# gauravchak/two_tower_models

Measured on AMD Instinct MI355X. Metric: user-item pairs/sec (in-batch softmax train step: fwd + zero_grad + bwd + dense-exact Adam), higher is better.
Workload: dtype f32

## Files before the change

### two_tower_models_amd/csrc/adam.hip

```cpp
#include <stdlib.h>

#include "common.hpp"

namespace tt {

constexpr int SWEEP_MAX_TABLES_DECL = 4;

constexpr int SWEEP_DEFAULT_PERSIST = 3;

struct AdamConst {
  float one_minus_b1, b2, one_minus_b2, eps, neg_step_size, inv_bc2_sqrt;
};

__device__ __forceinline__ AdamConst load_hyper(const double* __restrict__ h) {
  AdamConst c;
  c.one_minus_b1 = (float)(1.0 - h[1]);
  c.b2 = (float)h[2];
  c.one_minus_b2 = (float)(1.0 - h[2]);
  c.eps = (float)h[3];
  c.neg_step_size = (float)(-h[5]);
  c.inv_bc2_sqrt = (float)(1.0 / h[6]);
  return c;
}

// ... 352 lines not shown
  const AdamConst c = load_hyper(hyper);
  const unsigned n_chunks = tabs.first_chunk[tabs.n];
  __shared__ unsigned s_next[2];
  if (threadIdx.x == 0) s_next[0] = atomicAdd(&ctr[0], 1u);
  __syncthreads();
  unsigned ch = s_next[0];
  int par = 0;
  while (ch < n_chunks) {
    if (threadIdx.x == 0) s_next[par ^ 1] = atomicAdd(&ctr[0], 1u);
    int t = 0;
#pragma unroll
    for (int q = 1; q < SWEEP_MAX_TABLES; ++q)
      if (q < tabs.n && ch >= tabs.first_chunk[q]) t = q;
    float4* __restrict__ W = tabs.W[t];
    float4* __restrict__ M = tabs.M[t];
    float4* __restrict__ V = tabs.V[t];
    const int64_t n4 = tabs.n4[t];
    const int64_t base = (int64_t)(ch - tabs.first_chunk[t]) * (256 * ITERS) + threadIdx.x;
#pragma unroll UNR
    for (int k = 0; k < ITERS; ++k) {
      const int64_t i = base + (int64_t)k * 256;
      if (i >= n4) break;
      float4 p = sweep_load(W + i), m = sweep_load(M + i), v = sweep_load(V + i);
      adam_elem_zero_grad(p.x, m.x, v.x, c);
      adam_elem_zero_grad(p.y, m.y, v.y, c);
      adam_elem_zero_grad(p.z, m.z, v.z, c);
      adam_elem_zero_grad(p.w, m.w, v.w, c);
      sweep_store(p, W + i); sweep_store(m, M + i); sweep_store(v, V + i);
    }
    __syncthreads();
    par ^= 1;
    ch = s_next[par];
  }
  if (threadIdx.x == 0) {
    if (atomicAdd(&ctr[1], 1u) == gridDim.x - 1) {
      ctr[0] = 0;
      ctr[1] = 0;
      __threadfence();
    }
  }
}

struct SweepTablesMarked {
  SweepTables t;
  const unsigned* marks[SWEEP_MAX_TABLES];
  int sh[SWEEP_MAX_TABLES];
};
template <int ITERS, int PAIR>
__global__ __launch_bounds__(256) void adam_sweep_tables_marked_kernel(const SweepTablesMarked tm, const double* __restrict__ hyper,
                                                                       unsigned* __restrict__ ctr) {
  const AdamConst c = load_hyper(hyper);
  const unsigned n_chunks = tm.t.first_chunk[tm.t.n];
  __shared__ unsigned s_next[2];
  if (threadIdx.x == 0) s_next[0] = atomicAdd(&ctr[0], 1u);
  __syncthreads();
  unsigned ch = s_next[0];
  int par = 0;
  while (ch < n_chunks) {
    if (threadIdx.x == 0) s_next[par ^ 1] = atomicAdd(&ctr[0], 1u);
    const unsigned chu = __builtin_amdgcn_readfirstlane(ch);
    int t = 0;
#pragma unroll
    for (int q = 1; q < SWEEP_MAX_TABLES; ++q)
      if (q < tm.t.n && chu >= tm.t.first_chunk[q]) t = q;
    float4* __restrict__ W = tm.t.W[t];
    float4* __restrict__ M = tm.t.M[t];
    float4* __restrict__ V = tm.t.V[t];
    const int64_t n4 = tm.t.n4[t];
    const unsigned lc = chu - tm.t.first_chunk[t];
    const int sh = tm.sh[t];
    const int64_t r0 = (int64_t)lc * ((256 * ITERS) >> sh);
    const unsigned* __restrict__ mk = tm.marks[t];
    unsigned w0 = 0, w1 = 0, w2 = 0, w3 = 0;
    if (mk) {
      const unsigned* mw = mk + (r0 >> 5);
      w0 = mw[0]; w1 = mw[1]; w2 = mw[2]; w3 = mw[3];
    }
    const int64_t base = (int64_t)lc * (256 * ITERS) + threadIdx.x;
#pragma unroll
    for (int k = 0; k < ITERS; k += PAIR) {
      float4 p[PAIR], m[PAIR], v[PAIR];
      bool live[PAIR];
#pragma unroll
      for (int q = 0; q < PAIR; ++q) {
        const int64_t i = base + (int64_t)(k + q) * 256;
        const int64_t row = r0 + (((k + q) * 256 + (int)threadIdx.x) >> sh);
        const int wj = (int)((row >> 5) - (r0 >> 5));
        const unsigned word = wj == 0 ? w0 : wj == 1 ? w1 : wj == 2 ? w2 : w3;
        live[q] = i < n4 && !((word >> (row & 31)) & 1u);
      }
#pragma unroll
      for (int q = 0; q < PAIR; ++q) {
        const int64_t i = base + (int64_t)(k + q) * 256;
        if (live[q]) { p[q] = sweep_load(W + i); m[q] = sweep_load(M + i); v[q] = sweep_load(V + i); }
      }
#pragma unroll
      for (int q = 0; q < PAIR; ++q) {
        const int64_t i = base + (int64_t)(k + q) * 256;
        if (live[q]) {
          adam_elem_zero_grad(p[q].x, m[q].x, v[q].x, c);
          adam_elem_zero_grad(p[q].y, m[q].y, v[q].y, c);
          adam_elem_zero_grad(p[q].z, m[q].z, v[q].z, c);
          adam_elem_zero_grad(p[q].w, m[q].w, v[q].w, c);
          sweep_store(p[q], W + i); sweep_store(m[q], M + i); sweep_store(v[q], V + i);
        }
      }
    }
    __syncthreads();
    par ^= 1;
    ch = s_next[par];
  }
  if (threadIdx.x == 0) {
    if (atomicAdd(&ctr[1], 1u) == gridDim.x - 1) {
      ctr[0] = 0;
      ctr[1] = 0;
      __threadfence();
    }
  }
}

__global__ __launch_bounds__(256) void adam_mark_rows_kernel(const int64_t* __restrict__ ids, int64_t n_ids, int64_t n_rows,
                                                             unsigned* __restrict__ marks) {
  const int64_t i = (int64_t)blockIdx.x * 256 + threadIdx.x;
  if (i >= n_ids) return;
  const int64_t row = ids[i];
  if (row >= 0 && row < n_rows) atomicOr(&marks[row >> 5], 1u << (row & 31));
}

__global__ __launch_bounds__(256) void adam_sweep_scalar_kernel(float* __restrict__ W, float* __restrict__ M,
                                                                float* __restrict__ V, int64_t i0, int64_t n,
                                                                const double* __restrict__ hyper) {
  const AdamConst c = load_hyper(hyper);
  const int64_t stride = (int64_t)gridDim.x * blockDim.x;
  for (int64_t i = i0 + (int64_t)blockIdx.x * blockDim.x + threadIdx.x; i < n; i += stride) {
    float p = W[i], m = M[i], v = V[i];
    adam_elem_zero_grad(p, m, v, c);
    W[i] = p; M[i] = m; V[i] = v;
  }
}

__device__ __forceinline__ void replay_consts(AdamConst& c, const double* __restrict__ h, const float* __restrict__ tab,
                                              int64_t cap, int64_t j) {
  if (j < cap) {
    c.neg_step_size = tab[2 * j];
    c.inv_bc2_sqrt = tab[2 * j + 1];
  } else {
    double h5, h6;
    step_consts_from_doubles(h[0], h[1], h[2], (double)j, h5, h6);
    c.neg_step_size = (float)(-h5);
    c.inv_bc2_sqrt = (float)(1.0 / h6);
  }
}

template <int Q>
__device__ __forceinline__ void replay_row_q(float* __restrict__ W, float* __restrict__ M, float* __restrict__ V,
                                             int64_t row, int64_t dim, int32_t from, int32_t to,
                                             const double* __restrict__ hyper, const float* __restrict__ tab,
                                             int64_t cap, int lane) {
  AdamConst c = load_hyper(hyper);
  for (int64_t d0 = 0; d0 < dim; d0 += 64 * Q) {
    float p[Q], m[Q], v[Q];
    bool live = false;
#pragma unroll
    for (int q = 0; q < Q; ++q) {
      const int64_t d = d0 + lane + 64 * q;
      const int64_t at = row * dim + (d < dim ? d : dim - 1);
      p[q] = W[at]; m[q] = M[at]; v[q] = V[at];
      live = live || (d < dim && (m[q] != 0.f || v[q] != 0.f));
    }
    if (!__any(live)) continue;
    for (int32_t j = from + 1; j <= to; ++j) {
      replay_consts(c, hyper, tab, cap, j);
#pragma unroll
      for (int q = 0; q < Q; ++q) adam_elem_zero_grad(p[q], m[q], v[q], c);
    }
#pragma unroll
    for (int q = 0; q < Q; ++q) {
      const int64_t d = d0 + lane + 64 * q;
      if (d < dim) { W[row * dim + d] = p[q]; M[row * dim + d] = m[q]; V[row * dim + d] = v[q]; }
    }
  }
}
__device__ __forceinline__ void replay_row(float* __restrict__ W, float* __restrict__ M, float* __restrict__ V,
                                           int64_t row, int64_t dim, int32_t from, int32_t to,
                                           const double* __restrict__ hyper, const float* __restrict__ tab,
                                           int64_t cap, int lane) {
  from = __builtin_amdgcn_readfirstlane(from);
  to = __builtin_amdgcn_readfirstlane(to);
  if (dim <= 64) replay_row_q<1>(W, M, V, row, dim, from, to, hyper, tab, cap, lane);
  else if (dim <= 128) replay_row_q<2>(W, M, V, row, dim, from, to, hyper, tab, cap, lane);
  else replay_row_q<4>(W, M, V, row, dim, from, to, hyper, tab, cap, lane);
}

__global__ __launch_bounds__(256) void adam_catchup_ids_kernel(float* __restrict__ W, float* __restrict__ M,
                                                               float* __restrict__ V, int64_t n_rows, int64_t dim,
                                                               const int64_t* __restrict__ ids, int64_t n_ids,
                                                               int32_t* __restrict__ last_step,
                                                               const double* __restrict__ hyper, int offset,
                                                               const float* __restrict__ tab, int64_t cap) {
  const int64_t i = (int64_t)blockIdx.x * 4 + (threadIdx.x >> 6);
  if (i >= n_ids) return;
  const int lane = threadIdx.x & 63;
  const int64_t row = ids[i];
  if (row < 0 || row >= n_rows) return;
  const int32_t target = (int32_t)hyper[4] + offset;
  int32_t prev = 0;
  if (lane == 0) prev = atomicMax(&last_step[row], target);
  prev = __shfl(prev, 0, 64);
  if (prev >= target) return;
  replay_row(W, M, V, row, dim, prev, target, hyper, tab, cap, lane);
}

__global__ __launch_bounds__(256) void adam_catchup_plan_kernel(float* __restrict__ W, float* __restrict__ M,
                                                                float* __restrict__ V, int64_t n_rows, int64_t dim,
                                                                const int32_t* __restrict__ sorted_ids,
                                                                const int32_t* __restrict__ seg_begin,
                                                                const int32_t* __restrict__ n_unique,
                                                                int32_t* __restrict__ last_step,
                                                                const double* __restrict__ hyper, int offset, int mark,
                                                                const float* __restrict__ tab, int64_t cap) {
  const int64_t u = (int64_t)blockIdx.x * 4 + (threadIdx.x >> 6);
  if (u >= *n_unique) return;
  const int lane = threadIdx.x & 63;
  const int64_t row = sorted_ids[seg_begin[u]];
  if (row >= n_rows) return;
  const int32_t target = (int32_t)hyper[4] + offset;
  const int32_t prev = last_step[row];
  if (prev < target) replay_row(W, M, V, row, dim, prev, target, hyper, tab, cap, lane);
  if (lane == 0) last_step[row] = target + mark;
}

__global__ __launch_bounds__(256) void adam_flush_kernel(float* __restrict__ W, float* __restrict__ M,
                                                         float* __restrict__ V, int64_t n_rows, int64_t dim,
                                                         int32_t* __restrict__ last_step,
                                                         const double* __restrict__ hyper,
                                                         const float* __restrict__ tab, int64_t cap) {
  const int lane = threadIdx.x & 63;
  const int32_t target = (int32_t)hyper[4];
  const int64_t stride = (int64_t)gridDim.x * 4;
  for (int64_t row = (int64_t)blockIdx.x * 4 + (threadIdx.x >> 6); row < n_rows; row += stride) {
    const int32_t prev = last_step[row];
    if (prev >= target) continue;
    replay_row(W, M, V, row, dim, prev, target, hyper, tab, cap, lane);
    if (lane == 0) last_step[row] = target;
  }
}

constexpr int ADAM_BATCH = 64;
struct AdamBatch { tt_adam_tensor t[ADAM_BATCH]; };
__global__ __launch_bounds__(256) void adam_dense_kernel(const AdamBatch ts, const double* __restrict__ hyper) {
  const tt_adam_tensor t = ts.t[blockIdx.y];
  const AdamConst c = load_hyper(hyper);
  const int64_t stride = (int64_t)gridDim.x * blockDim.x;
  for (int64_t i = (int64_t)blockIdx.x * blockDim.x + threadIdx.x; i < t.n; i += stride) {
    float p = t.p[i], m = t.m[i], v = t.v[i];
    adam_elem(p, m, v, t.g[i], c);
    t.p[i] = p; t.m[i] = m; t.v[i] = v;
  }
}

__global__ __launch_bounds__(256) void pack_grads_kernel(const AdamBatch ts) {
  const tt_adam_tensor t = ts.t[blockIdx.y];
  const int64_t stride = (int64_t)gridDim.x * blockDim.x;
  for (int64_t i = (int64_t)blockIdx.x * blockDim.x + threadIdx.x; i < t.n; i += stride) t.p[i] = t.g[i];
}

__global__ __launch_bounds__(256) void copy_buffers_kernel(const AdamBatch ts) {
  const tt_adam_tensor t = ts.t[blockIdx.y];
  char* dst = reinterpret_cast<char*>(t.p);
  const char* src = reinterpret_cast<const char*>(t.g);
  const int64_t stride = (int64_t)gridDim.x * blockDim.x, i0 = (int64_t)blockIdx.x * blockDim.x + threadIdx.x;
  const bool vec = ((reinterpret_cast<uintptr_t>(dst) | reinterpret_cast<uintptr_t>(src)) & 15) == 0;
  const int64_t n16 = vec ? t.n / 16 : 0;
  for (int64_t i = i0; i < n16; i += stride) reinterpret_cast<uint4*>(dst)[i] = reinterpret_cast<const uint4*>(src)[i];
  for (int64_t i = n16 * 16 + i0; i < t.n; i += stride) dst[i] = src[i];
}

__global__ __launch_bounds__(256) void rowgrad_dense_kernel(const tt_grad_sources src, int64_t n_rows, int64_t dim,
                                                            const int32_t* __restrict__ sorted_ids,
                                                            const int32_t* __restrict__ perm,
                                                            const int32_t* __restrict__ seg_begin,
                                                            const int32_t* __restrict__ n_unique,
                                                            float* __restrict__ dense) {
  const int64_t u = (int64_t)blockIdx.x * 4 + (threadIdx.x >> 6);
  if (u >= *n_unique) return;
  const int lane = threadIdx.x & 63;
  const int32_t t0 = seg_begin[u], t1 = seg_begin[u + 1];
  const int64_t row = sorted_ids[t0];
  if (row >= n_rows) return;
  for (int64_t d = lane; d < dim; d += 64) {
    float g = 0.f;
    for (int32_t t = t0; t < t1; ++t) g += source_row(src, perm[t])[d];
    dense[row * dim + d] = g;
  }
}

static bool check_sources(const tt_grad_sources* s, int64_t n_ids, int64_t dim) {
  if (!s || s->n_sources < 1 || s->n_sources > TT_MAX_GRAD_SOURCES || s->first[0] != 0) return false;
  for (int k = 0; k < s->n_sources; ++k)
    if (!s->rows[k] || s->ld[k] < dim || s->first[k + 1] < s->first[k]) return false;
  return s->first[s->n_sources] == n_ids;
}

static int device_cu_count() {
  static int cached[64] = {0};
  int dev = 0;
  if (hipGetDevice(&dev) != hipSuccess || dev < 0 || dev >= 64) return 256;
  if (cached[dev] == 0) {
    int n = 0;
    cached[dev] = (hipDeviceGetAttribute(&n, hipDeviceAttributeMultiprocessorCount, dev) == hipSuccess && n > 0) ? n : 256;
  }
  return cached[dev];
}

static int launch_sweep(float* W, float* M, float* V, int64_t n_rows, int64_t dim, const double* hyper,
                        hipStream_t st, int n_wgs = 0) {
  int rc;
  const int64_t total = n_rows * dim;
  const bool vec = ((reinterpret_cast<uintptr_t>(W) | reinterpret_cast<uintptr_t>(M) | reinterpret_cast<uintptr_t>(V)) & 15) == 0;
  const int64_t n4 = vec ? total / 4 : 0;
  if (n4 > 0) {
    float4 *w4 = reinterpret_cast<float4*>(W), *m4 = reinterpret_cast<float4*>(M), *v4 = reinterpret_cast<float4*>(V);
    ProfScope prof("adam_sweep_kernel", st);
    unsigned* ctr = reinterpret_cast<unsigned*>(const_cast<double*>(hyper) + 7);
    unsigned grid = (unsigned)(device_cu_count() * SWEEP_DEFAULT_PERSIST);
    if (n_wgs > 0 && (unsigned)n_wgs < grid) grid = (unsigned)n_wgs;
    adam_sweep_persistent_kernel<4, 4><<<grid, 256, 0, st>>>(w4, m4, v4, n4, hyper, ctr);
    if ((rc = check_launch("adam_sweep_kernel"))) return rc;
  }
  if (n4 * 4 < total) {
    const int64_t rem = total - n4 * 4;
    const int64_t blocks = ceil_div(rem, 256) < 2048 ? ceil_div(rem, 256) : 2048;
    adam_sweep_scalar_kernel<<<(unsigned)blocks, 256, 0, st>>>(W, M, V, n4 * 4, total, hyper);
    if ((rc = check_launch("adam_sweep_scalar_kernel"))) return rc;
  }
  return 0;
}

}

using namespace tt;

extern "C" int tt_adam_advance(double* hyper, tt_stream_t stream) {
  if (!hyper) return fail_arg("tt_adam_advance: null pointer");
  adam_advance_kernel<<<1, 1, 0, S(stream)>>>(hyper, nullptr, 0);
  return check_launch("adam_advance_kernel");
}

extern "C" int64_t tt_adam_table_workspace_bytes(int64_t n_ids, int64_t dim) {
  if (n_ids <= 0 || dim <= 0) return 256;
  return round_up(n_ids * 3 * dim * 4, 256);
}

extern "C" int tt_adam_table(float* W, float* M, float* V, int64_t n_rows, int64_t dim, const double* hyper,
                             const tt_grad_sources* src, int64_t n_ids, const int32_t* sorted_ids,
                             const int32_t* perm, const int32_t* seg_begin, const int32_t* n_unique,
                             void* ws, int64_t ws_bytes, tt_stream_t stream) {
  if (!W || !M || !V || !hyper) return fail_arg("tt_adam_table: null pointer");
  if (n_rows <= 0 || dim <= 0 || n_ids < 0) return fail_arg("tt_adam_table: sizes");
  hipStream_t st = S(stream);
  int rc;
  if (n_ids > 0) {
    if (!sorted_ids || !perm || !seg_begin || !n_unique || !ws) return fail_arg("tt_adam_table: null plan");
    if (!check_sources(src, n_ids, dim)) return fail_arg("tt_adam_table: gradient sources");
    if (ws_bytes < tt_adam_table_workspace_bytes(n_ids, dim)) { set_error("tt_adam_table: workspace"); return TT_E_WORKSPACE; }
    adam_touched_kernel<false><<<(unsigned)ceil_div(n_ids, 4), 256, 0, st>>>(W, M, V, n_rows, dim, hyper, *src, sorted_ids, perm, seg_begin, n_unique, reinterpret_cast<float*>(ws), n_ids);
    if ((rc = check_launch("adam_touched_kernel"))) return rc;
  }
  if ((rc = launch_sweep(W, M, V, n_rows, dim, hyper, st))) return rc;
  if (n_ids > 0) {
    adam_writeback_kernel<<<(unsigned)ceil_div(n_ids, 4), 256, 0, st>>>(W, M, V, n_rows, dim, sorted_ids, seg_begin, perm, n_unique, reinterpret_cast<const float*>(ws), n_ids);
    if ((rc = check_launch("adam_writeback_kernel"))) return rc;
  }
  return 0;
}

extern "C" int tt_adam_table_stash(const float* W, const float* M, const float* V, int64_t n_rows, int64_t dim,
                                   int64_t n_ids, const int32_t* sorted_ids, const int32_t* perm,
                                   const int32_t* seg_begin, const int32_t* n_unique, void* side,
                                   int64_t side_bytes, tt_stream_t stream) {
  if (!W || !M || !V || !sorted_ids || !perm || !seg_begin || !n_unique || !side) return fail_arg("tt_adam_table_stash: null pointer");
  if (n_rows <= 0 || dim <= 0 || n_ids <= 0) return fail_arg("tt_adam_table_stash: sizes");
  if (side_bytes < tt_adam_table_workspace_bytes(n_ids, dim)) { set_error("tt_adam_table_stash: side buffer"); return TT_E_WORKSPACE; }
  adam_stash_kernel<<<(unsigned)ceil_div(n_ids, 4), 256, 0, S(stream)>>>(W, M, V, n_rows, dim, sorted_ids, seg_begin, perm, n_unique, reinterpret_cast<float*>(side), n_ids);
  return check_launch("adam_stash_kernel");
}

extern "C" int tt_adam_table_stash_ids(const float* W, const float* M, const float* V, int64_t n_rows, int64_t dim,
                                       const int64_t* ids, int64_t n_ids, void* side, int64_t side_bytes,
                                       tt_stream_t stream) {
  if (!W || !M || !V || !ids || !side) return fail_arg("tt_adam_table_stash_ids: null pointer");
  if (n_rows <= 0 || dim <= 0 || n_ids <= 0) return fail_arg("tt_adam_table_stash_ids: sizes");
  if (side_bytes < tt_adam_table_workspace_bytes(n_ids, dim)) { set_error("tt_adam_table_stash_ids: side buffer"); return TT_E_WORKSPACE; }
  adam_stash_ids_kernel<<<(unsigned)ceil_div(n_ids, 4), 256, 0, S(stream)>>>(W, M, V, n_rows, dim, ids, n_ids, reinterpret_cast<float*>(side));
  return check_launch("adam_stash_ids_kernel");
}

static int begin_ids_impl(double* hyper, float* tab, int64_t tab_steps, const tt_adam_stash_job* jobs, int32_t n_jobs, int planes,
                          tt_stream_t stream);

extern "C" int tt_adam_begin_ids(double* hyper, float* tab, int64_t tab_steps, const tt_adam_stash_job* jobs, int32_t n_jobs,
                                 tt_stream_t stream) {
  return begin_ids_impl(hyper, tab, tab_steps, jobs, n_jobs, 7, stream);
}

extern "C" int tt_adam_begin_ids_planes(double* hyper, float* tab, int64_t tab_steps, const tt_adam_stash_job* jobs, int32_t n_jobs,
                                        int32_t planes, tt_stream_t stream) {
  if (planes <= 0 || planes > 7) return fail_arg("tt_adam_begin_ids_planes: planes is a mask of 1 (p), 2 (m), 4 (v)");
  if (n_jobs > SWEEP_MAX_TABLES) return fail_arg("tt_adam_begin_ids_planes: at most 4 tables");
  return begin_ids_impl(hyper, tab, tab_steps, jobs, n_jobs, planes, stream);
}

static int begin_ids_impl(double* hyper, float* tab, int64_t tab_steps, const tt_adam_stash_job* jobs, int32_t n_jobs, int planes,
                          tt_stream_t stream) {
  if (!hyper || (n_jobs > 0 && !jobs) || n_jobs < 0) return fail_arg("tt_adam_begin_ids: null pointer");
  if (tab && tab_steps <= 0) return fail_arg("tt_adam_begin_ids: sizes");
  hipStream_t st = S(stream);
  if (n_jobs > SWEEP_MAX_TABLES) {
    int rc = tab ? tt_adam_advance_tab(hyper, tab, tab_steps, stream) : tt_adam_advance(hyper, stream);
    for (int i = 0; i < n_jobs && !rc; ++i)
      rc = tt_adam_table_stash_ids(jobs[i].W, jobs[i].M, jobs[i].V, jobs[i].n_rows, jobs[i].dim, jobs[i].ids, jobs[i].n_ids,
                                   jobs[i].side, jobs[i].side_bytes, stream);
    return rc;
  }
  StashJobs a{};
  a.n = n_jobs;
  unsigned blocks = 0;
  for (int i = 0; i < n_jobs; ++i) {
    const tt_adam_stash_job& j = jobs[i];
    if (!j.W || !j.M || !j.V || !j.ids || !j.side) return fail_arg("tt_adam_begin_ids: null pointer");
    if (j.n_rows <= 0 || j.dim <= 0 || j.n_ids <= 0) return fail_arg("tt_adam_begin_ids: sizes");
    if (j.side_bytes < tt_adam_table_workspace_bytes(j.n_ids, j.dim)) { set_error("tt_adam_begin_ids: side buffer"); return TT_E_WORKSPACE; }
    a.W[i] = j.W; a.M[i] = j.M; a.V[i] = j.V; a.ids[i] = j.ids; a.side[i] = reinterpret_cast<float*>(j.side);
    a.n_rows[i] = j.n_rows; a.dim[i] = j.dim; a.n_ids[i] = j.n_ids;
    a.first_block[i] = blocks;
    blocks += (unsigned)ceil_div(j.n_ids, 4);
  }
  for (int i = n_jobs; i <= SWEEP_MAX_TABLES; ++i) a.first_block[i] = blocks;
  adam_begin_ids_kernel<<<blocks + 1, 256, 0, st>>>(a, hyper, tab, tab ? tab_steps : 0, planes, planes & 1);
  return check_launch("adam_begin_ids_kernel");
}

extern "C" int tt_adam_table_sweep(float* W, float* M, float* V, int64_t n_rows, int64_t dim, const double* hyper,
                                   tt_stream_t stream) {
  if (!W || !M || !V || !hyper) return fail_arg("tt_adam_table_sweep: null pointer");
  if (n_rows <= 0 || dim <= 0) return fail_arg("tt_adam_table_sweep: sizes");
  return launch_sweep(W, M, V, n_rows, dim, hyper, S(stream));
}

extern "C" int tt_adam_tables_sweep(const tt_adam_tensor* tables, int32_t n_tables, const double* hyper, int32_t n_wgs,
                                    tt_stream_t stream) {
  if (!tables || !hyper) return fail_arg("tt_adam_tables_sweep: null pointer");
  if (n_tables <= 0 || n_tables > SWEEP_MAX_TABLES) return fail_arg("tt_adam_tables_sweep: 1..4 tables");
  hipStream_t st = S(stream);
  bool fused = n_tables > 1;
  SweepTables tabs{};
  unsigned chunks = 0;
  for (int t = 0; t < n_tables; ++t) {
    const tt_adam_tensor& d = tables[t];
    if (!d.p || !d.m || !d.v || d.n <= 0) return fail_arg("tt_adam_tables_sweep: descriptor");
    if (((reinterpret_cast<uintptr_t>(d.p) | reinterpret_cast<uintptr_t>(d.m) | reinterpret_cast<uintptr_t>(d.v)) & 15) || d.n % 4) fused = false;
    tabs.W[t] = reinterpret_cast<float4*>(d.p); tabs.M[t] = reinterpret_cast<float4*>(d.m); tabs.V[t] = reinterpret_cast<float4*>(d.v);
    tabs.n4[t] = d.n / 4;
    tabs.first_chunk[t] = chunks;
    const int64_t c = ceil_div(d.n / 4, 256 * 4);
    if (c + chunks >= (1ll << 32)) fused = false;
    chunks += (unsigned)c;
  }
  tabs.first_chunk[n_tables] = chunks;
  tabs.n = n_tables;
  static const int wgs_env = getenv("TT_SWEEP_WGS") ? atoi(getenv("TT_SWEEP_WGS")) : 0;
  const int want = getenv("TT_SWEEP_WGS") ? wgs_env : n_wgs;
  if (!fused) {
    for (int t = 0; t < n_tables; ++t) {
      const int rc = launch_sweep(tables[t].p, tables[t].m, tables[t].v, tables[t].n, 1, hyper, st, want);
      if (rc) return rc;
    }
    return 0;
  }
  unsigned* ctr = reinterpret_cast<unsigned*>(const_cast<double*>(hyper) + 7);
  unsigned grid = (unsigned)(device_cu_count() * SWEEP_DEFAULT_PERSIST);
  if (want > 0 && (unsigned)want < grid) grid = (unsigned)want;
  ProfScope prof("adam_sweep_kernel", st);
  adam_sweep_tables_kernel<4, 4><<<grid, 256, 0, st>>>(tabs, hyper, ctr);
  return check_launch("adam_sweep_tables_kernel");
}

extern "C" int64_t tt_adam_marks_words(int64_t n_rows) { return n_rows > 0 ? (n_rows + 31) / 32 + 4 : 4; }

extern "C" int tt_adam_mark_rows(const int64_t* ids, int64_t n_ids, int64_t n_rows, uint32_t* marks, int64_t marks_words,
                                 tt_stream_t stream) {
  if (!ids || !marks) return fail_arg("tt_adam_mark_rows: null pointer");
  if (n_ids <= 0 || n_rows <= 0) return fail_arg("tt_adam_mark_rows: sizes");
  if (marks_words < tt_adam_marks_words(n_rows)) { set_error("tt_adam_mark_rows: bitmap of %lld words < %lld", (long long)marks_words, (long long)tt_adam_marks_words(n_rows)); return TT_E_WORKSPACE; }
  hipStream_t st = S(stream);
  hipError_t e = hipMemsetAsync(marks, 0, (size_t)marks_words * 4, st);
  if (e != hipSuccess) { set_error("tt_adam_mark_rows: hipMemsetAsync: %s", hipGetErrorString(e)); return (int)e; }
  adam_mark_rows_kernel<<<(unsigned)ceil_div(n_ids, 256), 256, 0, st>>>(ids, n_ids, n_rows, marks);
  return check_launch("adam_mark_rows_kernel");
}

extern "C" int tt_adam_marked_supported(int64_t dim) {
  if (dim < 32 || dim > 4096 || (dim & (dim - 1))) return 0;
  return 1;
}

extern "C" int tt_adam_tables_sweep_marked(const tt_adam_tensor* tables, const int64_t* dims, const uint32_t* const* marks,
                                           int32_t n_tables, const double* hyper, int32_t n_wgs, tt_stream_t stream) {
  if (!tables || !dims || !marks || !hyper) return fail_arg("tt_adam_tables_sweep_marked: null pointer");
  if (n_tables <= 0 || n_tables > SWEEP_MAX_TABLES) return fail_arg("tt_adam_tables_sweep_marked: 1..4 tables");
  SweepTablesMarked tm{};
  unsigned chunks = 0;
  for (int t = 0; t < n_tables; ++t) {
    const tt_adam_tensor& d = tables[t];
    if (!d.p || !d.m || !d.v || d.n <= 0) return fail_arg("tt_adam_tables_sweep_marked: descriptor");
    if (!tt_adam_marked_supported(dims[t]) || d.n % dims[t]) return fail_arg("tt_adam_tables_sweep_marked: dim must be a power of two in [32, 4096]");
    if ((reinterpret_cast<uintptr_t>(d.p) | reinterpret_cast<uintptr_t>(d.m) | reinterpret_cast<uintptr_t>(d.v)) & 15)
      return fail_arg("tt_adam_tables_sweep_marked: 16-byte aligned tables");
    tm.t.W[t] = reinterpret_cast<float4*>(d.p); tm.t.M[t] = reinterpret_cast<float4*>(d.m); tm.t.V[t] = reinterpret_cast<float4*>(d.v);
    tm.t.n4[t] = d.n / 4;
    tm.t.first_chunk[t] = chunks;
    const int64_t c = ceil_div(d.n / 4, 256 * 4);
    if (c + chunks >= (1ll << 32)) return fail_arg("tt_adam_tables_sweep_marked: too many chunks");
    chunks += (unsigned)c;
    tm.marks[t] = marks[t];
    int sh = 0;
    while ((4ll << sh) < dims[t]) ++sh;
    tm.sh[t] = sh;
  }
  tm.t.first_chunk[n_tables] = chunks;
  tm.t.n = n_tables;
  static const int wgs_env = getenv("TT_SWEEP_WGS") ? atoi(getenv("TT_SWEEP_WGS")) : 0;
  const int want = getenv("TT_SWEEP_WGS") ? wgs_env : n_wgs;
  unsigned* ctr = reinterpret_cast<unsigned*>(const_cast<double*>(hyper) + 7);
  unsigned grid = (unsigned)(device_cu_count() * SWEEP_DEFAULT_PERSIST);
  if (want > 0 && (unsigned)want < grid) grid = (unsigned)want;
  hipStream_t st = S(stream);
  ProfScope prof("adam_sweep_kernel", st);
  adam_sweep_tables_marked_kernel<4, 2><<<grid, 256, 0, st>>>(tm, hyper, ctr);
  return check_launch("adam_sweep_tables_marked_kernel");
}

extern "C" int tt_stream_create_low_priority(void** out) {
  if (!out) return fail_arg("tt_stream_create_low_priority: null pointer");
  int least = 0, greatest = 0;
  hipError_t e = hipDeviceGetStreamPriorityRange(&least, &greatest);
  if (e != hipSuccess) { set_error("hipDeviceGetStreamPriorityRange: %s", hipGetErrorString(e)); return (int)e; }
  hipStream_t s;
  e = hipStreamCreateWithPriority(&s, hipStreamNonBlocking, least);
  if (e != hipSuccess) { set_error("hipStreamCreateWithPriority: %s", hipGetErrorString(e)); return (int)e; }
  *out = reinterpret_cast<void*>(s);
  return 0;
}
extern "C" int tt_stream_destroy(void* stream) {
  if (!stream) return 0;
  hipError_t e = hipStreamDestroy(reinterpret_cast<hipStream_t>(stream));
  if (e != hipSuccess) { set_error("hipStreamDestroy: %s", hipGetErrorString(e)); return (int)e; }
  return 0;
}

extern "C" int tt_adam_table_finish(float* W, float* M, float* V, int64_t n_rows, int64_t dim, const double* hyper,
                                    const tt_grad_sources* src, int64_t n_ids, const int32_t* sorted_ids,
                                    const int32_t* perm, const int32_t* seg_begin, const int32_t* n_unique,
                                    void* side, int64_t side_bytes, tt_stream_t stream) {
  if (!W || !M || !V || !hyper || !sorted_ids || !perm || !seg_begin || !n_unique)
    return fail_arg("tt_adam_table_finish: null pointer");
  if (n_rows <= 0 || dim <= 0 || n_ids <= 0) return fail_arg("tt_adam_table_finish: sizes");
  if (!check_sources(src, n_ids, dim)) return fail_arg("tt_adam_table_finish: gradient sources");
  if (side && side_bytes < tt_adam_table_workspace_bytes(n_ids, dim)) { set_error("tt_adam_table_finish: side buffer"); return TT_E_WORKSPACE; }
  hipStream_t st = S(stream);
  float* sd = reinterpret_cast<float*>(side);
  bool vec = dim % 4 == 0 && ((reinterpret_cast<uintptr_t>(W) | reinterpret_cast<uintptr_t>(M) | reinterpret_cast<uintptr_t>(V) |
                               reinterpret_cast<uintptr_t>(side)) & 15) == 0;
  for (int k = 0; vec && k < src->n_sources; ++k)
    vec = (reinterpret_cast<uintptr_t>(src->rows[k]) & 15) == 0 && src->ld[k] % 4 == 0;
  if (vec) {
    if (dim <= 64) adam_finish_kernel<16><<<(unsigned)ceil_div(n_ids, 16), 256, 0, st>>>(W, M, V, n_rows, dim, hyper, *src, sorted_ids, perm, seg_begin, n_unique, sd, n_ids);
    else if (dim <= 128) adam_finish_kernel<32><<<(unsigned)ceil_div(n_ids, 8), 256, 0, st>>>(W, M, V, n_rows, dim, hyper, *src, sorted_ids, perm, seg_begin, n_unique, sd, n_ids);
    else adam_finish_kernel<64><<<(unsigned)ceil_div(n_ids, 4), 256, 0, st>>>(W, M, V, n_rows, dim, hyper, *src, sorted_ids, perm, seg_begin, n_unique, sd, n_ids);
    return check_launch("adam_finish_kernel");
  }
  if (!side) return fail_arg("tt_adam_table_finish: marked rows (side == NULL) need dim % 4 == 0 and 16-byte aligned operands");
  adam_touched_kernel<true><<<(unsigned)ceil_div(n_ids, 4), 256, 0, st>>>(W, M, V, n_rows, dim, hyper, *src, sorted_ids, perm, seg_begin, n_unique, sd, n_ids);
  int rc = check_launch("adam_touched_kernel");
  if (rc) return rc;
  adam_writeback_kernel<<<(unsigned)ceil_div(n_ids, 4), 256, 0, st>>>(W, M, V, n_rows, dim, sorted_ids, seg_begin, perm, n_unique, sd, n_ids);
  return check_launch("adam_writeback_kernel");
}

extern "C" int tt_adam_tables_finish(const tt_adam_finish_job* jobs, int32_t n_jobs, const double* hyper, tt_stream_t stream) {
  if (!jobs || !hyper || n_jobs <= 0) return fail_arg("tt_adam_tables_finish: null pointer");
  bool one = n_jobs <= SWEEP_MAX_TABLES;
  int lpr = 0;
  for (int i = 0; i < n_jobs; ++i) {
    const tt_adam_finish_job& j = jobs[i];
    if (!j.W || !j.M || !j.V || !j.src || !j.sorted_ids || !j.perm || !j.seg_begin || !j.n_unique)
      return fail_arg("tt_adam_tables_finish: null pointer");
    if (j.n_rows <= 0 || j.dim <= 0 || j.n_ids <= 0) return fail_arg("tt_adam_tables_finish: sizes");
    if (!check_sources(j.src, j.n_ids, j.dim)) return fail_arg("tt_adam_tables_finish: gradient sources");
    if (j.side && j.side_bytes < tt_adam_table_workspace_bytes(j.n_ids, j.dim)) { set_error("tt_adam_tables_finish: side buffer"); return TT_E_WORKSPACE; }
    bool vec = j.dim % 4 == 0 && ((reinterpret_cast<uintptr_t>(j.W) | reinterpret_cast<uintptr_t>(j.M) | reinterpret_cast<uintptr_t>(j.V) |
                                   reinterpret_cast<uintptr_t>(j.side)) & 15) == 0;
    for (int k = 0; vec && k < j.src->n_sources; ++k)
      vec = (reinterpret_cast<uintptr_t>(j.src->rows[k]) & 15) == 0 && j.src->ld[k] % 4 == 0;
    const int cls = j.dim <= 64 ? 16 : j.dim <= 128 ? 32 : 64;
    if (!vec || (lpr && cls != lpr)) one = false;
    lpr = lpr ? lpr : cls;
  }
  if (!one) {
    for (int i = 0; i < n_jobs; ++i) {
      const tt_adam_finish_job& j = jobs[i];
      int rc = tt_adam_table_finish(j.W, j.M, j.V, j.n_rows, j.dim, hyper, j.src, j.n_ids, j.sorted_ids, j.perm, j.seg_begin,
                                    j.n_unique, j.side, j.side_bytes, stream);
      if (rc) return rc;
    }
    return 0;
  }
// ... 168 lines not shown
```

### two_tower_models_amd/csrc/attention_mfma.hip

```cpp
#include <stdlib.h>

#include "common.hpp"

namespace tt {

typedef float f32x16 __attribute__((ext_vector_type(16)));

constexpr int HP = 64;

__device__ __forceinline__ int arow(int e, int h) { return (e & 3) + 8 * (e >> 2) + 4 * h; }

template <int DH>
struct AttnLds {
  static constexpr int LD = DH + 4;
  static constexpr int MAT = HP * LD;
};

template <int DH>
__device__ __forceinline__ void stage(float* dst, const float* __restrict__ src, int64_t ld, int H, float scale, int lane) {
  constexpr int C4 = DH / 4, LD = DH + 4;
#pragma unroll
  for (int it = 0; it < HP * C4 / 64; ++it) {
    const int f = it * 64 + lane;
    const int row = f / C4, c4 = f % C4;
    const bool ok = row < H;
    const float* p = src + (int64_t)(ok ? row : H - 1) * ld + 4 * c4;
    const float x0 = p[0], x1 = p[1], x2 = p[2], x3 = p[3];
    const float4 v = make_float4(ok ? x0 * scale : 0.f, ok ? x1 * scale : 0.f, ok ? x2 * scale : 0.f, ok ? x3 * scale : 0.f);
    *reinterpret_cast<float4*>(dst + row * LD + 4 * c4) = v;
  }
}

template <int DH>
__device__ __forceinline__ void load_bfrag(float4 (&bf)[DH / 8], const float* __restrict__ src, int64_t ld, int row,
                                           int H, float scale, int h) {
  const bool ok = row < H;
  const float* p = src + (int64_t)(ok ? row : H - 1) * ld + 4 * h;
#pragma unroll
  for (int g = 0; g < DH / 8; ++g) {
    const float x0 = p[8 * g], x1 = p[8 * g + 1], x2 = p[8 * g + 2], x3 = p[8 * g + 3];
    bf[g] = make_float4(ok ? x0 * scale : 0.f, ok ? x1 * scale : 0.f, ok ? x2 * scale : 0.f, ok ? x3 * scale : 0.f);
  }
}
template <int DH>
__device__ __forceinline__ f32x16 nt_tile_rb(const float* A, int a0, const float4 (&bf)[DH / 8], int r, int h) {
  constexpr int LD = DH + 4;
  f32x16 acc;
#pragma unroll
  for (int e = 0; e < 16; ++e) acc[e] = 0.f;
  const float* ap = A + (a0 + r) * LD + 4 * h;
#pragma unroll
  for (int g = 0; g < DH / 8; ++g) {
    const float4 a = *reinterpret_cast<const float4*>(ap + 8 * g);
    acc = __builtin_amdgcn_mfma_f32_32x32x2f32(a.x, bf[g].x, acc, 0, 0, 0);
    acc = __builtin_amdgcn_mfma_f32_32x32x2f32(a.y, bf[g].y, acc, 0, 0, 0);
    acc = __builtin_amdgcn_mfma_f32_32x32x2f32(a.z, bf[g].z, acc, 0, 0, 0);
    acc = __builtin_amdgcn_mfma_f32_32x32x2f32(a.w, bf[g].w, acc, 0, 0, 0);
  }
  return acc;
}

template <int DH>
__device__ __forceinline__ void py_accum(f32x16 (&out)[(DH + 31) / 32], const f32x16& G, const float* Y, int y0,
                                         int r, int h) {
  constexpr int LD = DH + 4, TD = (DH + 31) / 32;
#pragma unroll
  for (int e = 0; e < 16; ++e) {
    const float* yrow = Y + (y0 + (e & 3) + 8 * (e >> 2) + 4 * h) * LD;
#pragma unroll
    for (int d = 0; d < TD; ++d) {
      const int col = 32 * d + r;
      const float yv = (DH % 32 == 0 || col < DH) ? yrow[col] : 0.f;
      out[d] = __builtin_amdgcn_mfma_f32_32x32x2f32(G[e], yv, out[d], 0, 0, 0);
    }
  }
}

template <int DH>
__device__ __forceinline__ void store_rows(float* __restrict__ dst, int64_t ld, const f32x16 (&t)[(DH + 31) / 32],
                                           int x0, int H, float scale, int r, int h) {
  constexpr int TD = (DH + 31) / 32;
#pragma unroll
  for (int d = 0; d < TD; ++d) {
    const int col = 32 * d + r;
    if (col >= DH) continue;
#pragma unroll
    for (int e = 0; e < 16; ++e) {
      const int row = x0 + arow(e, h);
      if (row < H) dst[(int64_t)row * ld + col] = t[d][e] * scale;
    }
  }
}

template <int DH, int WAVES>
__global__ __launch_bounds__(64 * WAVES, (WAVES == 4 ? 2 : 1)) void attn_fwd_mfma_kernel(const float* __restrict__ qkv, int64_t n_pairs,
                                                                   int H, int D, int heads,
                                                                   float* __restrict__ ctx, float* __restrict__ lse) {
  using L = AttnLds<DH>;
  constexpr int TD = (DH + 31) / 32;
  extern __shared__ __attribute__((aligned(16))) char smem_raw[];
  const int lane = threadIdx.x & 63, wave = threadIdx.x >> 6, r = lane & 31, h = lane >> 5;
  const int64_t pair = (int64_t)blockIdx.x * WAVES + wave;
  if (pair >= n_pairs) return;
  float* Ks = reinterpret_cast<float*>(smem_raw) + wave * 2 * L::MAT;
  float* Vs = Ks + L::MAT;
  const int64_t b = pair / heads, hd = pair % heads;
  const float* base = qkv + b * H * 3 * (int64_t)D + hd * DH;
  const float scale = 1.0f / sqrtf((float)DH);
  constexpr int C4 = DH / 4, NST = HP * C4 / 64;
  float4 kst[NST], vst[NST];
#pragma unroll
  for (int it = 0; it < NST; ++it) {
    const int f = it * 64 + lane, row = f / C4, c4 = f % C4;
    const float* pr = base + (int64_t)(row < H ? row : H - 1) * (3 * D) + 4 * c4;
    kst[it] = *reinterpret_cast<const float4*>(pr + D);
    vst[it] = *reinterpret_cast<const float4*>(pr + 2 * D);
  }
  float4 qf0[DH / 8], qf1[DH / 8];
  load_bfrag<DH>(qf0, base, 3 * D, r, H, scale, h);
  load_bfrag<DH>(qf1, base, 3 * D, 32 + r, H, scale, h);
#pragma unroll
  for (int it = 0; it < NST; ++it) {
    const int f = it * 64 + lane, row = f / C4, c4 = f % C4;
    const bool ok = row < H;
    float4 kv = kst[it], vv = vst[it];
    const float m = ok ? 1.f : 0.f;
    kv.x *= m; kv.y *= m; kv.z *= m; kv.w *= m;
    vv.x *= m; vv.y *= m; vv.z *= m; vv.w *= m;
    *reinterpret_cast<float4*>(Ks + row * L::LD + 4 * c4) = kv;
    *reinterpret_cast<float4*>(Vs + row * L::LD + 4 * c4) = vv;
  }
  __builtin_amdgcn_wave_barrier();

  float* out = ctx + b * H * (int64_t)D + hd * DH;
  auto query_tile = [&](int it, const float4 (&qf)[DH / 8]) {
    f32x16 st[2];
    float mx = -3.0e38f;
#pragma unroll
    for (int jt = 0; jt < 2; ++jt) {
      st[jt] = nt_tile_rb<DH>(Ks, jt * 32, qf, r, h);
#pragma unroll
      for (int e = 0; e < 16; ++e) {
        const bool valid = jt * 32 + arow(e, h) < H;
        st[jt][e] = valid ? st[jt][e] : -3.0e38f;
        mx = fmaxf(mx, st[jt][e]);
      }
    }
    mx = fmaxf(mx, __shfl_xor(mx, 32, 64));
    float l = 0.f;
#pragma unroll
    for (int jt = 0; jt < 2; ++jt)
#pragma unroll
      for (int e = 0; e < 16; ++e) {
        st[jt][e] = __expf(st[jt][e] - mx);
        l += st[jt][e];
      }
    l += __shfl_xor(l, 32, 64);
    const float inv = 1.0f / l;
    f32x16 o[TD];
#pragma unroll
    for (int d = 0; d < TD; ++d)
#pragma unroll
      for (int e = 0; e < 16; ++e) o[d][e] = 0.f;
#pragma unroll
    for (int jt = 0; jt < 2; ++jt) {
#pragma unroll
      for (int e = 0; e < 16; ++e) st[jt][e] *= inv;
      py_accum<DH>(o, st[jt], Vs, jt * 32, r, h);
    }
    store_rows<DH>(out, D, o, it * 32, H, 1.f, r, h);
    const int i = it * 32 + r;
    if (h == 0 && i < H) lse[(b * heads + hd) * H + i] = mx + __logf(l);
  };
  query_tile(0, qf0);
  query_tile(1, qf1);
}

template <int DH, int WAVES>
__global__ __launch_bounds__(64 * WAVES, (WAVES == 4 ? 2 : 1)) void attn_bwd_mfma_kernel(const float* __restrict__ qkv,
                                                                   const float* __restrict__ lse,
                                                                   const float* __restrict__ d_ctx, int64_t n_pairs,
                                                                   int H, int D, int heads,
                                                                   float* __restrict__ d_qkv) {
  using L = AttnLds<DH>;
  constexpr int TD = (DH + 31) / 32;
  constexpr int PER_WAVE = 2 * L::MAT + 2 * HP;
  extern __shared__ __attribute__((aligned(16))) char smem_raw[];
  const int lane = threadIdx.x & 63, wave = threadIdx.x >> 6, r = lane & 31, h = lane >> 5;
  const int64_t pair = (int64_t)blockIdx.x * WAVES + wave;
  if (pair >= n_pairs) return;
  float* M0 = reinterpret_cast<float*>(smem_raw) + wave * PER_WAVE;
  float* M1 = M0 + L::MAT;
  float* Ls = M1 + L::MAT;
  float* Ds = Ls + HP;
  const int64_t b = pair / heads, hd = pair % heads;
  const float* base = qkv + b * H * 3 * (int64_t)D + hd * DH;
  const float* gbase = d_ctx + b * H * (int64_t)D + hd * DH;
  const float scale = 1.0f / sqrtf((float)DH);
  float* Ks = M0;
  float* Vs = M1;
  stage<DH>(Ks, base + D, 3 * D, H, 1.f, lane);
  stage<DH>(Vs, base + 2 * D, 3 * D, H, 1.f, lane);
  Ls[lane] = (lane < H) ? lse[(b * heads + hd) * H + lane] : 3.0e38f;
  __builtin_amdgcn_wave_barrier();
  float* obase = d_qkv + b * H * 3 * (int64_t)D + hd * DH;

#pragma unroll
  for (int it = 0; it < 2; ++it) {
    const int i = it * 32 + r;
    const float li = Ls[i];
    float4 qf[DH / 8], gf[DH / 8];
    load_bfrag<DH>(qf, base, 3 * D, i, H, scale, h);
    load_bfrag<DH>(gf, gbase, D, i, H, 1.f, h);
    f32x16 pt[2], dpt[2];
    float dl = 0.f;
#pragma unroll
    for (int jt = 0; jt < 2; ++jt) {
      pt[jt] = nt_tile_rb<DH>(Ks, jt * 32, qf, r, h);
      dpt[jt] = nt_tile_rb<DH>(Vs, jt * 32, gf, r, h);
#pragma unroll
      for (int e = 0; e < 16; ++e) {
        const bool valid = jt * 32 + arow(e, h) < H;
        pt[jt][e] = valid ? __expf(pt[jt][e] - li) : 0.f;
        dl = fmaf(pt[jt][e], dpt[jt][e], dl);
      }
    }
    dl += __shfl_xor(dl, 32, 64);
    if (h == 0) Ds[i] = dl;
    f32x16 dq[TD];
#pragma unroll
    for (int d = 0; d < TD; ++d)
#pragma unroll
      for (int e = 0; e < 16; ++e) dq[d][e] = 0.f;
#pragma unroll
    for (int jt = 0; jt < 2; ++jt) {
#pragma unroll
      for (int e = 0; e < 16; ++e) pt[jt][e] *= (dpt[jt][e] - dl);
      py_accum<DH>(dq, pt[jt], Ks, jt * 32, r, h);
    }
    store_rows<DH>(obase, 3 * D, dq, it * 32, H, scale, r, h);
  }
  __builtin_amdgcn_wave_barrier();

  float* Qs = M0;
  float* Gs = M1;
  stage<DH>(Qs, base, 3 * D, H, scale, lane);
  stage<DH>(Gs, gbase, D, H, 1.f, lane);
  __builtin_amdgcn_wave_barrier();
#pragma unroll
  for (int jt = 0; jt < 2; ++jt) {
    const bool jvalid = jt * 32 + r < H;
    float4 kf[DH / 8], vf[DH / 8];
    load_bfrag<DH>(kf, base + D, 3 * D, jt * 32 + r, H, 1.f, h);
    load_bfrag<DH>(vf, base + 2 * D, 3 * D, jt * 32 + r, H, 1.f, h);
    f32x16 dv[TD], dk[TD];
#pragma unroll
    for (int d = 0; d < TD; ++d)
#pragma unroll
      for (int e = 0; e < 16; ++e) { dv[d][e] = 0.f; dk[d][e] = 0.f; }
#pragma unroll
    for (int it = 0; it < 2; ++it) {
      f32x16 p = nt_tile_rb<DH>(Qs, it * 32, kf, r, h);
      f32x16 dp = nt_tile_rb<DH>(Gs, it * 32, vf, r, h);
      const float* lrow = Ls + it * 32 + 4 * h;
      const float* drow = Ds + it * 32 + 4 * h;
#pragma unroll
      for (int q = 0; q < 4; ++q) {
        const float4 l4 = *reinterpret_cast<const float4*>(lrow + 8 * q);
        const float4 d4 = *reinterpret_cast<const float4*>(drow + 8 * q);
        const float lv[4] = {l4.x, l4.y, l4.z, l4.w}, dv4[4] = {d4.x, d4.y, d4.z, d4.w};
#pragma unroll
        for (int c = 0; c < 4; ++c) {
          const int e = 4 * q + c;
          const float pe = jvalid ? __expf(p[e] - lv[c]) : 0.f;
          p[e] = pe;
          dp[e] = pe * (dp[e] - dv4[c]);
        }
      }
      py_accum<DH>(dv, p, Gs, it * 32, r, h);
      py_accum<DH>(dk, dp, Qs, it * 32, r, h);
    }
    store_rows<DH>(obase + 2 * D, 3 * D, dv, jt * 32, H, 1.f, r, h);
    store_rows<DH>(obase + D, 3 * D, dk, jt * 32, H, 1.f, r, h);
  }
}

template <typename K>
static int lds_opt_in(K kernel, size_t lds, const char* name) {
  if (lds <= 64 * 1024) return 0;
  hipError_t e = hipFuncSetAttribute(reinterpret_cast<const void*>(kernel), hipFuncAttributeMaxDynamicSharedMemorySize, (int)lds);
  if (e != hipSuccess) { set_error("%s: hipFuncSetAttribute: %s", name, hipGetErrorString(e)); return (int)e; }
  return 0;
}

template <int DH>
static int launch_fwd(const float* qkv, int64_t n_pairs, int H, int D, int heads, float* ctx, float* lse, hipStream_t st) {
  constexpr int WAVES = 4;
  const size_t lds = (size_t)WAVES * 2 * AttnLds<DH>::MAT * sizeof(float);
  int rc = lds_opt_in(attn_fwd_mfma_kernel<DH, WAVES>, lds, "attn_fwd_mfma_kernel");
  if (rc) return rc;
  ProfScope prof("attn_fwd_mfma_kernel", st);
  attn_fwd_mfma_kernel<DH, WAVES><<<(unsigned)ceil_div(n_pairs, WAVES), 64 * WAVES, lds, st>>>(qkv, n_pairs, H, D, heads, ctx, lse);
  return check_launch("attn_fwd_mfma_kernel");
}
template <int DH>
static int launch_bwd(const float* qkv, const float* lse, const float* d_ctx, int64_t n_pairs, int H, int D, int heads,
                      float* d_qkv, hipStream_t st) {
  constexpr int WAVES = (DH <= 32) ? 4 : 2;
  const size_t lds = (size_t)WAVES * (2 * AttnLds<DH>::MAT + 2 * HP) * sizeof(float);
  int rc = lds_opt_in(attn_bwd_mfma_kernel<DH, WAVES>, lds, "attn_bwd_mfma_kernel");
  if (rc) return rc;
  ProfScope prof("attn_bwd_mfma_kernel", st);
  attn_bwd_mfma_kernel<DH, WAVES><<<(unsigned)ceil_div(n_pairs, WAVES), 64 * WAVES, lds, st>>>(qkv, lse, d_ctx, n_pairs, H, D, heads, d_qkv);
  return check_launch("attn_bwd_mfma_kernel");
}

bool attn_mfma_supported(const void* a, const void* b, int64_t H, int64_t D, int64_t dh) {
  const bool al = ((reinterpret_cast<uintptr_t>(a) | reinterpret_cast<uintptr_t>(b)) & 15) == 0;
  return al && H <= HP && (dh == 16 || dh == 32 || dh == 64) && D % 4 == 0;
}

int attn_fwd_mfma(const float* qkv, int64_t B, int64_t H, int64_t D, int64_t heads, float* ctx, float* lse, hipStream_t st) {
  const int64_t dh = D / heads, n = B * heads;
  if (dh == 16) return launch_fwd<16>(qkv, n, (int)H, (int)D, (int)heads, ctx, lse, st);
  if (dh == 32) return launch_fwd<32>(qkv, n, (int)H, (int)D, (int)heads, ctx, lse, st);
  return launch_fwd<64>(qkv, n, (int)H, (int)D, (int)heads, ctx, lse, st);
}
int attn_bwd_mfma(const float* qkv, const float* lse, const float* d_ctx, int64_t B, int64_t H, int64_t D,
                  int64_t heads, float* d_qkv, hipStream_t st) {
  const int64_t dh = D / heads, n = B * heads;
  if (dh == 16) return launch_bwd<16>(qkv, lse, d_ctx, n, (int)H, (int)D, (int)heads, d_qkv, st);
  if (dh == 32) return launch_bwd<32>(qkv, lse, d_ctx, n, (int)H, (int)D, (int)heads, d_qkv, st);
  return launch_bwd<64>(qkv, lse, d_ctx, n, (int)H, (int)D, (int)heads, d_qkv, st);
}

}
```

### two_tower_models_amd/csrc/common.hpp

```cpp
#pragma once
#include <hip/hip_runtime.h>
#include <stdint.h>
#include <stdio.h>

#include "../../include/tt_hotpath.h"

namespace tt {

void set_error(const char* fmt, ...);

inline int fail_arg(const char* what) {
  set_error("bad argument: %s", what);
  return TT_E_BADARG;
}

inline int check_launch(const char* kernel) {
  hipError_t e = hipGetLastError();
  if (e != hipSuccess) {
    set_error("%s: %s", kernel, hipGetErrorString(e));
    return (int)e;
  }
  return 0;
}

inline hipStream_t S(tt_stream_t s) { return reinterpret_cast<hipStream_t>(s); }

struct ProfScope {
  ProfScope(const char* name, hipStream_t st);
  ~ProfScope();
  hipStream_t st_;
  int slot_, idx_;
};

constexpr int WAVE = 64;

inline int64_t ceil_div(int64_t a, int64_t b) { return (a + b - 1) / b; }
inline int64_t round_up(int64_t a, int64_t b) { return ceil_div(a, b) * b; }

struct Carver {
  char* base;
  int64_t off = 0;
  explicit Carver(void* p) : base(reinterpret_cast<char*>(p)) {}
  template <typename T>
  T* take(int64_t count) {
    T* p = reinterpret_cast<T*>(base + off);
    off += round_up(count * (int64_t)sizeof(T), 256);
    return p;
  }
};

__device__ __forceinline__ float wave_sum(float v) {
#pragma unroll
  for (int o = 32; o > 0; o >>= 1) v += __shfl_xor(v, o, 64);
  return v;
}
__device__ __forceinline__ float wave_max(float v) {
#pragma unroll
  for (int o = 32; o > 0; o >>= 1) v = fmaxf(v, __shfl_xor(v, o, 64));
  return v;
}

}
```

Before: 1.524 million.

## Make attention forward persistent with buffer loads prefetching the next pair

```diff
diff --git a/two_tower_models_amd/csrc/adam.hip b/two_tower_models_amd/csrc/adam.hip
--- a/two_tower_models_amd/csrc/adam.hip
+++ b/two_tower_models_amd/csrc/adam.hip
@@ -678,17 +678,6 @@
   return s->first[s->n_sources] == n_ids;
 }
 
-static int device_cu_count() {
-  static int cached[64] = {0};
-  int dev = 0;
-  if (hipGetDevice(&dev) != hipSuccess || dev < 0 || dev >= 64) return 256;
-  if (cached[dev] == 0) {
-    int n = 0;
-    cached[dev] = (hipDeviceGetAttribute(&n, hipDeviceAttributeMultiprocessorCount, dev) == hipSuccess && n > 0) ? n : 256;
-  }
-  return cached[dev];
-}
-
 static int launch_sweep(float* W, float* M, float* V, int64_t n_rows, int64_t dim, const double* hyper,
                         hipStream_t st, int n_wgs = 0) {
   int rc;
diff --git a/two_tower_models_amd/csrc/attention_mfma.hip b/two_tower_models_amd/csrc/attention_mfma.hip
--- a/two_tower_models_amd/csrc/attention_mfma.hip
+++ b/two_tower_models_amd/csrc/attention_mfma.hip
@@ -93,87 +93,153 @@
 }
 
 template <int DH, int WAVES>
-__global__ __launch_bounds__(64 * WAVES, (WAVES == 4 ? 2 : 1)) void attn_fwd_mfma_kernel(const float* __restrict__ qkv, int64_t n_pairs,
-                                                                   int H, int D, int heads,
-                                                                   float* __restrict__ ctx, float* __restrict__ lse) {
+__device__ __forceinline__ void attn_fwd_pairs(const float* __restrict__ qkv, int64_t n_pairs, int H, int D, int heads,
+                                               float* __restrict__ ctx, float* __restrict__ lse) {
   using L = AttnLds<DH>;
   constexpr int TD = (DH + 31) / 32;
   extern __shared__ __attribute__((aligned(16))) char smem_raw[];
-  const int lane = threadIdx.x & 63, wave = threadIdx.x >> 6, r = lane & 31, h = lane >> 5;
-  const int64_t pair = (int64_t)blockIdx.x * WAVES + wave;
+  const int lane = threadIdx.x & 63, r = lane & 31, h = lane >> 5;
+  const int wave = __builtin_amdgcn_readfirstlane(threadIdx.x >> 6);
+  int64_t pair = (int64_t)blockIdx.x * WAVES + wave;
   if (pair >= n_pairs) return;
+  const int64_t stride = (int64_t)gridDim.x * WAVES;
+  const int db = (int)stride / heads, dhd = (int)stride % heads;
+  int64_t b = (int)pair / heads;
+  int hd = (int)pair % heads;
   float* Ks = reinterpret_cast<float*>(smem_raw) + wave * 2 * L::MAT;
   float* Vs = Ks + L::MAT;
-  const int64_t b = pair / heads, hd = pair % heads;
-  const float* base = qkv + b * H * 3 * (int64_t)D + hd * DH;
   const float scale = 1.0f / sqrtf((float)DH);
   constexpr int C4 = DH / 4, NST = HP * C4 / 64;
-  float4 kst[NST], vst[NST];
+  const int qrow0 = r < H ? r : H - 1, qrow1 = 32 + r < H ? 32 + r : H - 1;
+
+  float4 kst[NST], vst[NST], qf0[DH / 8], qf1[DH / 8];
+  unsigned kvoff[NST];
 #pragma unroll
   for (int it = 0; it < NST; ++it) {
     const int f = it * 64 + lane, row = f / C4, c4 = f % C4;
-    const float* pr = base + (int64_t)(row < H ? row : H - 1) * (3 * D) + 4 * c4;
-    kst[it] = *reinterpret_cast<const float4*>(pr + D);
-    vst[it] = *reinterpret_cast<const float4*>(pr + 2 * D);
-  }
-  float4 qf0[DH / 8], qf1[DH / 8];
-  load_bfrag<DH>(qf0, base, 3 * D, r, H, scale, h);
-  load_bfrag<DH>(qf1, base, 3 * D, 32 + r, H, scale, h);
-#pragma unroll
-  for (int it = 0; it < NST; ++it) {
-    const int f = it * 64 + lane, row = f / C4, c4 = f % C4;
-    const bool ok = row < H;
-    float4 kv = kst[it], vv = vst[it];
-    const float m = ok ? 1.f : 0.f;
-    kv.x *= m; kv.y *= m; kv.z *= m; kv.w *= m;
-    vv.x *= m; vv.y *= m; vv.z *= m; vv.w *= m;
-    *reinterpret_cast<float4*>(Ks + row * L::LD + 4 * c4) = kv;
-    *reinterpret_cast<float4*>(Vs + row * L::LD + 4 * c4) = vv;
-  }
-  __builtin_amdgcn_wave_barrier();
-
-  float* out = ctx + b * H * (int64_t)D + hd * DH;
-  auto query_tile = [&](int it, const float4 (&qf)[DH / 8]) {
-    f32x16 st[2];
-    float mx = -3.0e38f;
-#pragma unroll
-    for (int jt = 0; jt < 2; ++jt) {
-      st[jt] = nt_tile_rb<DH>(Ks, jt * 32, qf, r, h);
-#pragma unroll
-      for (int e = 0; e < 16; ++e) {
-        const bool valid = jt * 32 + arow(e, h) < H;
-        st[jt][e] = valid ? st[jt][e] : -3.0e38f;
-        mx = fmaxf(mx, st[jt][e]);
+    kvoff[it] = 4u * (unsigned)((row < H ? row : H - 1) * (3 * D) + 4 * c4);
+  }
+  const unsigned qoff0 = 4u * (unsigned)(qrow0 * (3 * D) + 4 * h), qoff1 = 4u * (unsigned)(qrow1 * (3 * D) + 4 * h);
+  const unsigned ooff = 4u * (unsigned)(4 * h * D + r);
+  const int pair_bytes = 4 * (H * 3 * D - DH * (heads - 1));
+  auto ld128 = [](__amdgpu_buffer_rsrc_t rs, unsigned voff, int soff) {
+    return __builtin_bit_cast(float4, __builtin_amdgcn_raw_buffer_load_b128(rs, (int)voff, soff, 0));
+  };
+  auto issue_kv = [&](__amdgpu_buffer_rsrc_t rs) {
+#pragma unroll
+    for (int it = 0; it < NST; ++it) {
+      kst[it] = ld128(rs, kvoff[it], 4 * D);
+      vst[it] = ld128(rs, kvoff[it], 8 * D);
+    }
+  };
+  auto issue_q = [&](float4 (&qf)[DH / 8], __amdgpu_buffer_rsrc_t rs, unsigned qoff) {
+#pragma unroll
+    for (int g = 0; g < DH / 8; ++g) qf[g] = ld128(rs, qoff, 32 * g);
+  };
+  auto pair_rsrc = [&](int64_t b_, int hd_) {
+    return __builtin_amdgcn_make_buffer_rsrc(const_cast<float*>(qkv + b_ * H * 3 * (int64_t)D + hd_ * DH), 0, pair_bytes, 0x00020000);
+  };
+  auto write_kv = [&]() {
+#pragma unroll
+    for (int it = 0; it < NST; ++it) {
+      const int f = it * 64 + lane, row = f / C4, c4 = f % C4;
+      float4 kv = kst[it], vv = vst[it];
+      const float m = row < H ? 1.f : 0.f;
+      kv.x *= m; kv.y *= m; kv.z *= m; kv.w *= m;
+      vv.x *= m; vv.y *= m; vv.z *= m; vv.w *= m;
+      *reinterpret_cast<float4*>(Ks + row * L::LD + 4 * c4) = kv;
+      *reinterpret_cast<float4*>(Vs + row * L::LD + 4 * c4) = vv;
+    }
+  };
+
+  const __amdgpu_buffer_rsrc_t rs = pair_rsrc(b, hd);
+  issue_kv(rs);
+  issue_q(qf0, rs, qoff0);
+  issue_q(qf1, rs, qoff1);
+  for (;;) {
+    write_kv();
+    const bool more = __builtin_amdgcn_readfirstlane((int)(pair + stride < n_pairs)) != 0;
+    int64_t nb = b + db;
+    int nhd = hd + dhd;
+    if (nhd >= heads) { nhd -= heads; ++nb; }
+    if (!more) { nb = b; nhd = hd; }
+    const __amdgpu_buffer_rsrc_t nrs = pair_rsrc(nb, nhd);
+    issue_kv(nrs);
+    __builtin_amdgcn_wave_barrier();
+
+    const __amdgpu_buffer_rsrc_t ors =
+        __builtin_amdgcn_make_buffer_rsrc(ctx + b * H * (int64_t)D + hd * DH, 0, 4 * (H * D - DH * (heads - 1)), 0x00020000);
+    float* lrow = lse + pair * H;
+    auto query_tile = [&](int it, float4 (&qf)[DH / 8], unsigned qoff) {
+      const bool qok = it * 32 + r < H;
+#pragma unroll
+      for (int g = 0; g < DH / 8; ++g)
+        qf[g] = make_float4(qok ? qf[g].x * scale : 0.f, qok ? qf[g].y * scale : 0.f, qok ? qf[g].z * scale : 0.f, qok ? qf[g].w * scale : 0.f);
+      f32x16 st[2];
+      float mx = -3.0e38f;
+#pragma unroll
+      for (int jt = 0; jt < 2; ++jt) {
+        st[jt] = nt_tile_rb<DH>(Ks, jt * 32, qf, r, h);
+#pragma unroll
+        for (int e = 0; e < 16; ++e) {
+          const bool valid = jt * 32 + arow(e, h) < H;
+          st[jt][e] = valid ? st[jt][e] : -3.0e38f;
+          mx = fmaxf(mx, st[jt][e]);
+        }
       }
-    }
-    mx = fmaxf(mx, __shfl_xor(mx, 32, 64));
-    float l = 0.f;
-#pragma unroll
-    for (int jt = 0; jt < 2; ++jt)
-#pragma unroll
-      for (int e = 0; e < 16; ++e) {
-        st[jt][e] = __expf(st[jt][e] - mx);
-        l += st[jt][e];
+      issue_q(qf, nrs, qoff);
+      mx = fmaxf(mx, __shfl_xor(mx, 32, 64));
+      float l = 0.f;
+#pragma unroll
+      for (int jt = 0; jt < 2; ++jt)
+#pragma unroll
+        for (int e = 0; e < 16; ++e) {
+          st[jt][e] = __expf(st[jt][e] - mx);
+          l += st[jt][e];
+        }
+      l += __shfl_xor(l, 32, 64);
+      const float inv = 1.0f / l;
+      f32x16 o[TD];
+#pragma unroll
+      for (int d = 0; d < TD; ++d)
+#pragma unroll
+        for (int e = 0; e < 16; ++e) o[d][e] = 0.f;
+#pragma unroll
+      for (int jt = 0; jt < 2; ++jt) {
+#pragma unroll
+        for (int e = 0; e < 16; ++e) st[jt][e] *= inv;
+        py_accum<DH>(o, st[jt], Vs, jt * 32, r, h);
       }
-    l += __shfl_xor(l, 32, 64);
-    const float inv = 1.0f / l;
-    f32x16 o[TD];
-#pragma unroll
-    for (int d = 0; d < TD; ++d)
-#pragma unroll
-      for (int e = 0; e < 16; ++e) o[d][e] = 0.f;
-#pragma unroll
-    for (int jt = 0; jt < 2; ++jt) {
-#pragma unroll
-      for (int e = 0; e < 16; ++e) st[jt][e] *= inv;
-      py_accum<DH>(o, st[jt], Vs, jt * 32, r, h);
-    }
-    store_rows<DH>(out, D, o, it * 32, H, 1.f, r, h);
-    const int i = it * 32 + r;
-    if (h == 0 && i < H) lse[(b * heads + hd) * H + i] = mx + __logf(l);
-  };
-  query_tile(0, qf0);
-  query_tile(1, qf1);
+#pragma unroll
+      for (int d = 0; d < TD; ++d) {
+        if (32 * d + r >= DH) continue;
+#pragma unroll
+        for (int e = 0; e < 16; ++e) {
+          const int row0 = it * 32 + (e & 3) + 8 * (e >> 2);
+          const float x = o[d][e];
+          if (row0 + 4 * h < H) __builtin_amdgcn_raw_buffer_store_b32(__builtin_bit_cast(unsigned, x), ors, (int)ooff, 4 * (row0 * D + 32 * d), 0);
+        }
+      }
+      const int i = it * 32 + r;
+      if (h == 0 && i < H) lrow[i] = mx + __logf(l);
+    };
+    query_tile(0, qf0, qoff0);
+    query_tile(1, qf1, qoff1);
+    if (!more) break;
+    __builtin_amdgcn_wave_barrier();
+    pair += stride; b = nb; hd = nhd;
+  }
+}
+
+template <int DH, int WAVES>
+__global__ __launch_bounds__(64 * WAVES, 2) __attribute__((amdgpu_num_vgpr(112))) void attn_fwd_mfma_kernel(
+    const float* __restrict__ qkv, int64_t n_pairs, int H, int D, int heads, float* __restrict__ ctx, float* __restrict__ lse) {
+  attn_fwd_pairs<DH, WAVES>(qkv, n_pairs, H, D, heads, ctx, lse);
+}
+template <>
+__global__ __launch_bounds__(256, 1) __attribute__((amdgpu_num_vgpr(256))) void attn_fwd_mfma_kernel<64, 4>(const float* __restrict__ qkv, int64_t n_pairs, int H, int D,
+                                                                     int heads, float* __restrict__ ctx, float* __restrict__ lse) {
+  attn_fwd_pairs<64, 4>(qkv, n_pairs, H, D, heads, ctx, lse);
 }
 
 template <int DH, int WAVES>
@@ -299,8 +365,9 @@
   const size_t lds = (size_t)WAVES * 2 * AttnLds<DH>::MAT * sizeof(float);
   int rc = lds_opt_in(attn_fwd_mfma_kernel<DH, WAVES>, lds, "attn_fwd_mfma_kernel");
   if (rc) return rc;
+  const int64_t blocks = ceil_div(n_pairs, WAVES), cap = 2 * (int64_t)device_cu_count();
   ProfScope prof("attn_fwd_mfma_kernel", st);
-  attn_fwd_mfma_kernel<DH, WAVES><<<(unsigned)ceil_div(n_pairs, WAVES), 64 * WAVES, lds, st>>>(qkv, n_pairs, H, D, heads, ctx, lse);
+  attn_fwd_mfma_kernel<DH, WAVES><<<(unsigned)(blocks < cap ? blocks : cap), 64 * WAVES, lds, st>>>(qkv, n_pairs, H, D, heads, ctx, lse);
   return check_launch("attn_fwd_mfma_kernel");
 }
 template <int DH>
diff --git a/two_tower_models_amd/csrc/common.hpp b/two_tower_models_amd/csrc/common.hpp
--- a/two_tower_models_amd/csrc/common.hpp
+++ b/two_tower_models_amd/csrc/common.hpp
@@ -34,6 +34,17 @@
 
 constexpr int WAVE = 64;
 
+inline int device_cu_count() {
+  static int cached[64] = {0};
+  int dev = 0;
+  if (hipGetDevice(&dev) != hipSuccess || dev < 0 || dev >= 64) return 256;
+  if (cached[dev] == 0) {
+    int n = 0;
+    cached[dev] = (hipDeviceGetAttribute(&n, hipDeviceAttributeMultiprocessorCount, dev) == hipSuccess && n > 0) ? n : 256;
+  }
+  return cached[dev];
+}
+
 inline int64_t ceil_div(int64_t a, int64_t b) { return (a + b - 1) / b; }
 inline int64_t round_up(int64_t a, int64_t b) { return ceil_div(a, b) * b; }
 
```

Result: no change. 1.534 million (median of 2 runs) (+0.6%).
